# HyHuang1995/gmmloc

Hardware: AMD Instinct MI355X
Metric: frames/sec (associate+pose-refine), 2k pts x 4k GMM (higher is better)
Workload: dtype f64

## Files before the change

gmmloc_amd/csrc/gl_ba.hip:

```cpp
#include <algorithm>
#include <cstdlib>
#include <cstring>

#include "gl_ba_common.hpp"

#pragma clang fp contract(fast)

using namespace gld;
using namespace glba;

namespace {

GL_DEV void point_solve(const PtLin& o, double lambda, double* f, double* b, double* u) {
  double D[6];
#pragma unroll
  for (int i = 0; i < 6; ++i) D[i] = o.A[i] + o.Hc[i];
  D[0] += lambda;
  D[3] += lambda;
  D[5] += lambda;
  ldl3_factor(D, f);
#pragma unroll
  for (int i = 0; i < 3; ++i) b[i] = o.a[i] + o.bc[i];
  ldl3_solve(f, b, u);
}
// ... 380 lines not shown
    if (!pose_fixed) se3_store(T, pose_io + (size_t)f * 7);
    if (iters_out) iters_out[f] = it3;
  }
}

}

namespace gl {

bool ba1_fast_supported(int L);
int launch_ba1_fast(Ctx* c, const Gmm* g, const gl_camera* cam, const gl_params* prm, int B, int L, double* pose,
                    double* pts, const double* obs, const int32_t* oct, int32_t* assoc, const double* d2, double gate,
                    uint8_t* dropped, uint8_t* erase, int32_t* iters, char* scratch, const Ba1Layout& lay, const uint8_t* prior,
                    const TrackFixed* fixed);

int track_frames_fixed(gl_ctx_t* ctx, const gl_gmm_t* gmm, const gl_camera* cam, const gl_params* prm, int B, int M,
                       double* pose_dev, double* Xw_dev, const double* obs_dev, const int32_t* octave_dev, int32_t* assoc_dev,
                       double* d2_dev, const gl_track_anchor* anchor);

int launch_ba1(Ctx* c, const Gmm* g, const gl_camera* cam, const gl_params* prm, int B, int L, double* pose,
               const uint8_t* has_prior, double* pts, const double* obs, const int32_t* oct, int32_t* assoc,
               const double* d2, double gate, uint8_t* dropped, uint8_t* erase, int32_t* iters, char* scratch, const Ba1Layout& lay) {
  BaK k = make_bak(cam, prm, gate);
  GmmDev gm{g->rec12, g->axis, g->sqrt_info, g->hgw, g->flags, g->plane4};
  {
    TimerScope ts(c, GL_TIMER_BA);
    k_ba1<<<B, T_BA, 0, c->stream>>>(k, gm, B, L, pose, has_prior, pts, obs, oct, assoc, d2, (double*)(scratch + lay.trial),
                                     (double*)(scratch + lay.chi), (uint8_t*)(scratch + lay.lev), dropped, erase, iters);
  }
  GL_HIP(hipGetLastError());
  return GL_OK;
}

}

static int track_frames_impl(gl_ctx_t* ctx, const gl_gmm_t* gmm, const gl_camera* cam, const gl_params* prm, int B, int M,
                             double* pose_dev, double* Xw_dev, const double* obs_dev, const int32_t* octave_dev,
                             int32_t* assoc_dev, double* d2_dev, const uint8_t* prior_dev, const gl::TrackFixed* fixed = nullptr) {
  GL_REQUIRE(ctx && gmm && cam && prm, "null argument");
  if (B == 0 || M == 0) return GL_OK;
  GL_REQUIRE(B > 0 && M > 0, "bad B / M");
  GL_REQUIRE(pose_dev && Xw_dev && obs_dev && octave_dev && assoc_dev, "null buffer");
  gl::Ctx* c = gl::C(ctx);
  gl::Gmm* g = gl::G(gmm);
  GL_HIP(hipSetDevice(c->device));
  const size_t n = (size_t)B * M;
  const bool fast = (c->opt.ba_slow == 0 || fixed) && gl::ba1_fast_supported(M);
  gl::Ba1Layout lay;
  int rc = gl::ba1_layout(c, B, M, fixed ? fixed->F : 0, prior_dev != nullptr, fast, &lay);
  if (rc != GL_OK) return rc;
  const bool use_grid = g->grid.enabled && c->opt.assoc_grid != 0;
  const size_t assoc_bytes =
      use_grid ? gl::assoc_index_scratch_bytes(g->K, (int)n, d2_dev != nullptr) : gl::assoc_scratch_bytes(g->K, (int)n);
  gl::Regions r{0};
  r.take(std::max(assoc_bytes, lay.end));
  const size_t o_d2 = r.take(n * 8);
  void* scratch = nullptr;
  rc = gl::ctx_scratch(c, r.off, &scratch);
  if (rc != GL_OK) return rc;
  double* d2 = d2_dev ? d2_dev : (double*)((char*)scratch + o_d2);
  if (use_grid)
    rc = gl::launch_assoc_index(c, g, Xw_dev, (int)n, assoc_dev, d2, d2_dev != nullptr, scratch);
  else
    rc = gl::launch_assoc_brute(c, g, Xw_dev, (int)n, assoc_dev, d2);
  if (rc != GL_OK) return rc;
  if (fast)
    return gl::launch_ba1_fast(c, g, cam, prm, B, M, pose_dev, Xw_dev, obs_dev, octave_dev, assoc_dev, d2, 9.0,
                               nullptr, nullptr, nullptr, (char*)scratch, lay, prior_dev, fixed);
  return gl::launch_ba1(c, g, cam, prm, B, M, pose_dev, prior_dev, Xw_dev, obs_dev, octave_dev, assoc_dev, d2, 9.0,
                        nullptr, nullptr, nullptr, (char*)scratch, lay);
}

extern "C" int gl_track_frames(gl_ctx_t* ctx, const gl_gmm_t* gmm, const gl_camera* cam, const gl_params* prm, int B,
                               int M, double* pose_dev, double* Xw_dev, const double* obs_dev,
                               const int32_t* octave_dev, int32_t* assoc_dev, double* d2_dev) {
  return track_frames_impl(ctx, gmm, cam, prm, B, M, pose_dev, Xw_dev, obs_dev, octave_dev, assoc_dev, d2_dev, nullptr);
}

extern "C" int gl_track_frames_anchored(gl_ctx_t* ctx, const gl_gmm_t* gmm, const gl_camera* cam, const gl_params* prm, int B,
                                        int M, double* pose_dev, double* Xw_dev, const double* obs_dev,
                                        const int32_t* octave_dev, int32_t* assoc_dev, double* d2_dev,
                                        const gl_track_anchor* anchor) {
  GL_REQUIRE(anchor, "null anchor");
  GL_REQUIRE(anchor->F >= 0 && anchor->F <= GL_TRACK_MAX_FIXED, "bad number of fixed observer key-frames");
  if (anchor->F == 0)
    return track_frames_impl(ctx, gmm, cam, prm, B, M, pose_dev, Xw_dev, obs_dev, octave_dev, assoc_dev, d2_dev, anchor->prior_dev);
  GL_REQUIRE(anchor->fixed_pose_dev && anchor->fixed_obs_dev && anchor->fixed_oct_dev, "null buffer of the fixed observer key-frames");
  if (ctx && anchor->F <= 4 && gl::ba1_fast_supported(M) && gl::C(ctx)->opt.ba_fixed_pack == 0 && gl::C(ctx)->opt.ba_slow == 0) {
    const gl::TrackFixed fx{anchor->F, anchor->fixed_pose_dev, anchor->fixed_obs_dev, anchor->fixed_oct_dev, anchor->fixed_erase_dev};
    return track_frames_impl(ctx, gmm, cam, prm, B, M, pose_dev, Xw_dev, obs_dev, octave_dev, assoc_dev, d2_dev, anchor->prior_dev, &fx);
  }
  return gl::track_frames_fixed(ctx, gmm, cam, prm, B, M, pose_dev, Xw_dev, obs_dev, octave_dev, assoc_dev, d2_dev, anchor);
}

static int track_frame_host_impl(gl_ctx_t* ctx, const gl_gmm_t* gmm, const gl_camera* cam, const gl_params* prm, int M,
                                 double* pose_host, double* Xw_host, const double* obs_host, const int32_t* octave_host,
                                 int32_t* assoc_host, int with_prior) {
  GL_REQUIRE(ctx && gmm && cam && prm, "null argument");
  GL_REQUIRE(M >= 0, "bad M");
  if (M == 0) return GL_OK;
  GL_REQUIRE(pose_host && Xw_host && obs_host && octave_host && assoc_host, "null buffer");
  gl::Ctx* c = gl::C(ctx);
  GL_HIP(hipSetDevice(c->device));
  const size_t oX = 64, oA = oX + (size_t)M * 24, oO = oA + (((size_t)M * 4 + 7) / 8) * 8, oC = oO + (size_t)M * 24,
               total = oC + (size_t)M * 4;
  if (c->stage_bytes < total) {
    GL_HIP(hipStreamSynchronize(c->stream));
    if (c->dev_stage) GL_HIP(hipFree(c->dev_stage));
    if (c->host_stage) GL_HIP(hipHostFree(c->host_stage));
    c->dev_stage = c->host_stage = nullptr;
    c->stage_bytes = 0;
    const size_t want = total + total / 4 + 64;
    GL_HIP(hipMalloc(&c->dev_stage, want));
    GL_HIP(hipHostMalloc(&c->host_stage, want, hipHostMallocDefault));
    c->stage_bytes = want;
  }
  char* st = (char*)c->host_stage;
  char* dv = (char*)c->dev_stage;
  memcpy(st, pose_host, 56);
  st[56] = with_prior ? 1 : 0;
  memcpy(st + oX, Xw_host, (size_t)M * 24);
  memcpy(st + oO, obs_host, (size_t)M * 24);
// ... 28 lines not shown
```

gmmloc_amd/csrc/gl_ba_fast.hip:

```cpp
#include <algorithm>
#include <cstdlib>

#include "gl_ba_common.hpp"

using namespace gld;
using namespace glba;

namespace {
struct PrepView {
  double* gobn;
  int32_t* perm;
  int32_t* pfl;
  int32_t* assoc_p;
};
struct FixedV {
  int F;
  double* fRt;
  double* fobn;
  int32_t* foct;
  double* chif;
  uint8_t* ferase;
};
struct BafKArgs {
  glba::BaK k;
  glba::GmmDev gm;
  int B, L, G, S;
  double* pose_io;
  double* pts_io;
  int32_t* assoc_all;
  uint8_t* dropped_all;
  uint8_t* erase_all;
  int32_t* iters_out;
  double* pn_all;
  int32_t* trials_out;
  int NB;
  unsigned long long* parts;
  int* ctl;
  long long limit;
  int xcc_trusted;
  const int32_t* oct_all;
  const uint8_t* prior_all;
  double* prior_mi;
  double* stage;
  int nb_prev;
  int32_t* counters;
  int32_t* outer_out;
  FixedV fxv;
  int32_t* edges_out;
  int* frame_ctr;
};
__host__ __device__ inline PrepView prep_view(double* scratch, int B, int L) {
  PrepView v;
  const size_t n = (size_t)B * L;
  v.gobn = scratch;
  v.perm = (int32_t*)(scratch + n * 3);
  v.pfl = v.perm + n;
  v.assoc_p = v.pfl + n;
  return v;
}

constexpr int PREP_T = 256, PREP_C = 8;
__global__ __launch_bounds__(PREP_T) void k_ba1_prep(BafKArgs A, const double* __restrict__ obs_all, const double* __restrict__ d2_all,
                                                    gl::TrackFixed fin, int* __restrict__ frame_ctr) {
  __shared__ int cnt[PREP_C][PREP_T / 64];
  __shared__ int cnt0[PREP_C][PREP_T / 64];
  const BaK& k = A.k;
  const int B = A.B, L = A.L, F = A.fxv.F;
  const int32_t* const oct_all = A.oct_all;
  int32_t* const assoc_all = A.assoc_all;
  const int f = blockIdx.x, tid = threadIdx.x, lane = tid & 63, wave = tid >> 6;
  if (f >= B) return;
  if (f == 0 && tid == 0) *frame_ctr = 0;
  if (A.parts) {
    const int nxw = 2 * A.G * 64;
    for (int i = tid; i < nxw; i += PREP_T) A.parts[(size_t)f * nxw + i] = 0ull;
    if (tid < 2) A.ctl[2 * f + tid] = 0;
  }
  if (A.prior_all && A.prior_all[f] && tid == 0) {
    const SE3 Ti = se3_inverse(se3_load(A.pose_io + (size_t)f * 7));
    double Ri[9];
    qtoR(Ti.r, Ri);
#pragma unroll
    for (int i = 0; i < 9; ++i) A.prior_mi[(size_t)f * 12 + i] = Ri[i];
#pragma unroll
    for (int i = 0; i < 3; ++i) A.prior_mi[(size_t)f * 12 + 9 + i] = Ti.t[i];
  }
  if (F > 0 && tid < F) {
    const SE3 T = se3_load(fin.pose + ((size_t)f * F + tid) * 7);
    double Rm[9];
    qtoR(T.r, Rm);
    double* o = A.fxv.fRt + ((size_t)f * F + tid) * 12;
#pragma unroll
    for (int i = 0; i < 9; ++i) o[i] = Rm[i];
#pragma unroll
    for (int i = 0; i < 3; ++i) o[9 + i] = T.t[i];
  }
  const size_t gbase = (size_t)f * L;
  const PrepView pv = prep_view(A.pn_all, B, L);
  const int rounds = (L + PREP_T - 1) / PREP_T;
  int a_[PREP_C], fl_[PREP_C];
#pragma unroll
  for (int j = 0; j < PREP_C; ++j) {
// ... 26 lines not shown
  __syncthreads();
  int total = 0, total0 = 0;
#pragma unroll
  for (int j = 0; j < PREP_C; ++j)
#pragma unroll
    for (int w = 0; w < PREP_T / 64; ++w) {
      total += cnt[j][w];
      total0 += cnt0[j][w];
    }
  const int n_others = L - total - total0, n_exist = L - total0;
  const double ifx = 1.0 / k.fx, ify = 1.0 / k.fy;
  int base = 0, base0 = 0;
#pragma unroll
  for (int j = 0; j < PREP_C; ++j) {
#pragma unroll
    for (int w = 0; w < PREP_T / 64; ++w)
      if (w < wave) {
        base += cnt[j][w];
        base0 += cnt0[j][w];
      }
    const int l = j * PREP_T + tid;
    const bool isnd = (fl_[j] & 12) == 4;
    const bool isempty = fl_[j] == 0 && j < rounds && l < L;
    const unsigned long long bal = __ballot(isnd), bal0 = __ballot(isempty);
    const int before = base + __popcll(bal & ((1ull << lane) - 1ull));
    const int before0 = base0 + __popcll(bal0 & ((1ull << lane) - 1ull));
    if (j < rounds && l < L) {
      const int lp = isempty ? n_exist + before0 : isnd ? n_others + before : l - before - before0;
      const size_t g = gbase + l, gp = gbase + lp;
      pv.perm[gp] = l;
      pv.pfl[gp] = fl_[j];
      pv.assoc_p[gp] = a_[j];
      pv.gobn[gp * 3] = (obs_all[g * 3] - k.cx) * ifx;
      pv.gobn[gp * 3 + 1] = (obs_all[g * 3 + 1] - k.cy) * ify;
      pv.gobn[gp * 3 + 2] = (obs_all[g * 3 + 2] - k.cx) * ifx;
      for (int kf = 0; kf < F; ++kf) {
        const size_t src = g * F + kf, dst = ((size_t)f * F + kf) * L + lp;
        const int fo = fl_[j] ? fin.oct[src] : -1;
        const double u = fin.obs[src * 3], v = fin.obs[src * 3 + 1], ur = fin.obs[src * 3 + 2];
        A.fxv.fobn[dst * 3] = (u - k.cx) * ifx;
        A.fxv.fobn[dst * 3 + 1] = (v - k.cy) * ify;
        A.fxv.fobn[dst * 3 + 2] = (ur - k.cx) * ifx;
        A.fxv.foct[dst] = fo < 0 ? -1 : ((fo & 7) | (!(ur < 0) ? 16 : 0));
        A.fxv.chif[dst] = 0.0;
      }
    }
#pragma unroll
    for (int w = 0; w < PREP_T / 64; ++w)
      if (w >= wave) {
        base += cnt[j][w];
        base0 += cnt0[j][w];
      }
  }
}
}

namespace {
struct BafCfg {
  int mcap, nw;
  bool spread, step32, prior, fixed;
};
namespace bafd2000 { constexpr BafCfg kCfg{2000, 8, false, false, false, false}; }
namespace bafs { constexpr BafCfg kCfg{256, 8, true, false, false, false}; }
#ifndef GL_BAF_QUICK
namespace bafd496 { constexpr BafCfg kCfg{496, 2, false, false, false, false}; }
namespace bafd1000 { constexpr BafCfg kCfg{1000, 4, false, false, false, false}; }
namespace bafs32 { constexpr BafCfg kCfg{256, 8, true, true, false, false}; }
namespace bafd2000s32 { constexpr BafCfg kCfg{2000, 8, false, true, false, false}; }
namespace bafd496p { constexpr BafCfg kCfg{496, 2, false, false, true, false}; }
namespace bafd1000p { constexpr BafCfg kCfg{992, 4, false, false, true, false}; }
namespace bafd2000p { constexpr BafCfg kCfg{2000, 8, false, false, true, false}; }
namespace bafsp { constexpr BafCfg kCfg{256, 8, true, false, true, false}; }
namespace bafd496f { constexpr BafCfg kCfg{496, 2, false, false, true, true}; }
namespace bafd1000f { constexpr BafCfg kCfg{984, 4, false, false, true, true}; }
namespace bafd2000f { constexpr BafCfg kCfg{2000, 8, false, false, true, true}; }
#endif
}
#define GL_BAF_NS bafd2000
#include "gl_ba_fast_impl.hpp"
#define GL_BAF_NS bafs
#include "gl_ba_fast_impl.hpp"
#ifndef GL_BAF_QUICK
#define GL_BAF_NS bafd496
#include "gl_ba_fast_impl.hpp"
#define GL_BAF_NS bafd1000
#include "gl_ba_fast_impl.hpp"
#define GL_BAF_NS bafs32
#include "gl_ba_fast_impl.hpp"
#define GL_BAF_NS bafd2000s32
#include "gl_ba_fast_impl.hpp"
#define GL_BAF_NS bafd496p
#include "gl_ba_fast_impl.hpp"
#define GL_BAF_NS bafd1000p
#include "gl_ba_fast_impl.hpp"
#define GL_BAF_NS bafd2000p
#include "gl_ba_fast_impl.hpp"
#define GL_BAF_NS bafsp
#include "gl_ba_fast_impl.hpp"
#define GL_BAF_NS bafd496f
#include "gl_ba_fast_impl.hpp"
#define GL_BAF_NS bafd1000f
#include "gl_ba_fast_impl.hpp"
#define GL_BAF_NS bafd2000f
#include "gl_ba_fast_impl.hpp"
namespace {
__device__ __forceinline__ int xcc_id() { return __builtin_amdgcn_s_getreg(20 | (0 << 6) | (3 << 11)) & 15; }
// ... 126 lines not shown
  in->kern<<<grid, threads, in->lds, c->stream>>>(a);
  GL_HIP(hipGetLastError());
  return GL_OK;
}

static int launch_spread(Ctx* c, BafKArgs a) {
  const BafInst* in = baf_instance(c, true, a.prior_all != nullptr, 0, 64 * a.S);
  GL_REQUIRE(in, "no refine instance for this launch");
  GL_HIP(ensure_dynamic_lds(c, (const void*)in->kern, in->lds));
  a.NB = a.G;
  a.limit = (long long)(c->opt.ba_rendezvous_us * 100.0);
  if (c->opt.ba_test_abort_seq > 0) a.limit = -(long long)c->opt.ba_test_abort_seq;
  a.xcc_trusted = (c->xcc_ids_trusted && c->opt.ba_same_xcd != 0) ? 1 : 0;
  const int grid = a.NB > 1 ? 64 * ((a.B + 7) / 8) : a.B;
  in->kern<<<grid, 256, in->lds, c->stream>>>(a);
  GL_HIP(hipGetLastError());
  return GL_OK;
}

int launch_ba1_fast(Ctx* c, const Gmm* g, const gl_camera* cam, const gl_params* prm, int B, int L, double* pose,
                    double* pts, const double* obs, const int32_t* oct, int32_t* assoc, const double* d2, double gate,
                    uint8_t* dropped, uint8_t* erase, int32_t* iters, char* scratch, const Ba1Layout& lay, const uint8_t* prior,
                    const TrackFixed* fixed) {
  BafKArgs a{};
  a.k = make_bak(cam, prm, gate);
  a.gm = GmmDev{g->rec12, g->axis, g->sqrt_info, g->hgw, g->flags, g->plane4};
  a.B = B;
  a.L = L;
  canon_order(L, &a.G, &a.S);
  a.pose_io = pose;
  a.pts_io = pts;
  a.assoc_all = assoc;
  a.dropped_all = dropped;
  a.erase_all = erase;
  a.iters_out = iters;
  a.pn_all = (double*)(scratch + lay.rec);
  a.trials_out = (c->stats && c->stats_n >= B) ? c->stats : nullptr;
  a.NB = 1;
  a.oct_all = oct;
  a.prior_all = prior;
  a.prior_mi = (double*)(scratch + lay.prior_mi);
  a.counters = c->counters;
  a.outer_out = a.trials_out ? c->stats_iters : nullptr;
  if (fixed)
    a.fxv = FixedV{fixed->F, (double*)(scratch + lay.frt), (double*)(scratch + lay.fobn), (int32_t*)(scratch + lay.foct),
                   (double*)(scratch + lay.chif), fixed->erase};
  a.edges_out = (c->stats_edges && c->stats_edges_n >= B) ? c->stats_edges : nullptr;
  if (lay.spread) {
    a.parts = (unsigned long long*)(scratch + lay.parts);
    a.ctl = (int*)(scratch + lay.ctl);
    a.stage = (double*)(scratch + lay.stage);
  }
  int* const frame_ctr = (int*)(scratch + lay.frame_ctr);
  {
    TimerScope ts(c, GL_TIMER_BA_PREP);
    k_ba1_prep<<<B, PREP_T, 0, c->stream>>>(a, obs, d2, fixed ? *fixed : TrackFixed{}, frame_ctr);
  }
  GL_HIP(hipGetLastError());
  TimerScope ts(c, GL_TIMER_BA);
  if (!lay.spread) return launch_dense(c, a, frame_ctr);
  const int rc = launch_spread(c, a);
  if (rc != GL_OK || a.G == 1) return rc;
  a.nb_prev = a.G;
  return launch_dense(c, a, frame_ctr);
}

}
#endif
```

gmmloc_amd/csrc/gl_ba_fast_impl.hpp:

```cpp
namespace {
namespace GL_BAF_NS {

constexpr int MCAP = kCfg.mcap;
constexpr bool kSpread = kCfg.spread;
constexpr bool kStep32 = kCfg.step32;
constexpr bool kPrior = kCfg.prior;
constexpr bool kFixed = kCfg.fixed;
constexpr int NWC = kCfg.nw;
constexpr int NRED = kSpread ? 1 : NWC;
constexpr int TSP = 256;
constexpr bool kLean = !kPrior;

#ifdef GL_BA_TRACE
__device__ double g_trace[10 * 128];
#define TRACE_TRIAL(t, a, b, c_, d, dxp)                            \
  if (blockIdx.x == 0 && threadIdx.x == 0 && (t) < 128) {            \
    g_trace[(t)*10] = (a);                                           \
    g_trace[(t)*10 + 1] = (b);                                       \
    g_trace[(t)*10 + 2] = (c_);                                      \
    g_trace[(t)*10 + 3] = (d);                                       \
    for (int i_ = 0; i_ < 6; ++i_) g_trace[(t)*10 + 4 + i_] = (dxp)[i_]; \
  }
#else
#define TRACE_TRIAL(t, a, b, c_, d, dxp)
// ... 1582 lines not shown
    est[0] += est[2] * (trials - est[3]);
    est[1] += est[2] * cj;
  }
  return cj;
}

template <class T>
GL_DEV T ld_karg(const T __attribute__((address_space(4)))* p) {
  static_assert(sizeof(T) % 4 == 0, "");
  union U {
    T v;
    unsigned w[sizeof(T) / 4];
    GL_DEV U() {}
  } u;
  const unsigned __attribute__((address_space(4)))* q = (const unsigned __attribute__((address_space(4)))*)p;
#pragma unroll
  for (unsigned i = 0; i < sizeof(T) / 4; ++i) u.w[i] = q[i];
  return u.v;
}

GL_DEV bool false_once_inlined() { return false; }

constexpr int kPriorWorkOwn = (kPrior && !kSpread && NWC < 4) ? 108 : 0;
constexpr int kLdsSp = 0;
constexpr int kLdsChir = kLdsSp + 3 * MCAP;
constexpr int kLdsUn = kLdsChir + MCAP;
constexpr int kLdsRed = kLdsUn + 6 * MCAP;
constexpr int kLdsTot = kLdsRed + NRED * 32;
constexpr int kLdsStab = kLdsTot + 64;
constexpr int kLdsRed2 = kLdsStab + 24;
constexpr int kLdsPrec = kLdsRed2 + (NWC > 8 ? 2 * NWC : 16);
constexpr int kLdsFrt = kLdsPrec + (kPrior ? 64 : 0) + kPriorWorkOwn;
constexpr int kLdsTb = kLdsFrt + (kFixed ? kMaxFixed * 12 : 0);
constexpr size_t kLdsBytes = (kLdsTb + (kSpread ? 29 * TSP : 0)) * sizeof(double);

typedef const BafKArgs __attribute__((address_space(4))) kargs_t;
GL_DEV void ba1_fast_frame(double* smem, const unsigned fblock, kargs_t* ka) {
  const BaK __attribute__((address_space(4)))& k = ka->k;
  const GmmDev gm = ld_karg(&ka->gm);
  const FixedV fxv = ld_karg(&ka->fxv);
  const int B = ka->B, L = ka->L, G = ka->G, S = ka->S, NB = ka->NB, xcc_trusted = ka->xcc_trusted, nb_prev = ka->nb_prev;
  double* const pose_io = ka->pose_io;
  double* const pts_io = ka->pts_io;
  int32_t* const assoc_all = ka->assoc_all;
  double* const pn_all = ka->pn_all;
  unsigned long long* const parts = ka->parts;
  int* const ctl = ka->ctl;
  const long long limit = ka->limit;
  const int32_t* const oct_all = ka->oct_all;
  const uint8_t* const prior_all = ka->prior_all;
  const double* const prior_mi = ka->prior_mi;
  double* const stage = ka->stage;
  int32_t* const counters = ka->counters;
  Lds D;
  D.sp = smem + kLdsSp;
  D.chir = smem + kLdsChir;
  D.un = smem + kLdsUn;
  Red R;
  R.red = smem + kLdsRed;
  R.tot = smem + kLdsTot;
  D.stab = smem + kLdsStab;
  R.red2 = smem + kLdsRed2;
  double* const prec = smem + kLdsPrec;
  D.frt = smem + kLdsFrt;
  R.tb = smem + kLdsTb;
  double* const pwork = kSpread ? R.tb + 2 * TSP : (NWC >= 4 ? R.red : prec + 64);
  D.F = 0;
  D.Lf = L;
  D.gfobn = nullptr;
  D.gfoct = nullptr;
  D.gchif = nullptr;
  R.S = S;
  FlagW fw = {0ull, 0u};
  const int tid = threadIdx.x, lane = tid & 63, wave = tid >> 6;
  PROF_K(0);
#ifdef GL_BA_PROF
  if (blockIdx.x == 1024 && threadIdx.x == 0) g_prof_k[12] = 0;
  const unsigned long long prof_wg_t0 = wall_clock64();
#endif
  const int f = kSpread ? (NB > 1 ? (int)(fblock & 7) + 8 * (int)(fblock >> 6) : (int)fblock) : (int)fblock;
  const int pb_ = kSpread && NB > 1 ? (int)((fblock >> 3) & 7) : 0;
  if (f >= B || pb_ >= NB) return;
  double* const st_pts = stage;
  double* const st_pose = stage ? stage + (size_t)B * L * 3 : nullptr;
  int32_t* const st_assoc = stage ? (int32_t*)(st_pose + (size_t)B * 8) : nullptr;
  if (!kSpread && ctl) {
    if (ctl[2 * f + 1] == nb_prev) {
      const int32_t* oc = oct_all + (size_t)f * L;
      const int NT = blockDim.x;
      for (int l0 = threadIdx.x; l0 < L; l0 += 4 * NT) {
        int o_[4], a_[4];
        double p_[4][3];
#pragma unroll
        for (int q = 0; q < 4; ++q) {
          const int l = min(l0 + q * NT, L - 1);
          const size_t g = (size_t)f * L + l;
          o_[q] = oc[l];
          a_[q] = st_assoc[g];
#pragma unroll
          for (int j = 0; j < 3; ++j) p_[q][j] = st_pts[g * 3 + j];
        }
#pragma unroll
        for (int q = 0; q < 4; ++q) {
          const int l = l0 + q * NT;
          if (l >= L) break;
          const size_t g = (size_t)f * L + l;
// ... 2 lines not shown
            for (int j = 0; j < 3; ++j) pts_io[g * 3 + j] = p_[q][j];
          }
          assoc_all[g] = a_[q];
        }
      }
      if (threadIdx.x < 7) pose_io[(size_t)f * 7 + threadIdx.x] = st_pose[(size_t)f * 8 + threadIdx.x];
      return;
    }
    if (counters && threadIdx.x == 0) atomicAdd(&counters[0], 1);
  }
  Coop C{kSpread && NB > 1 ? parts + (size_t)f * 2 * NB * 64 : nullptr, kSpread ? NB : 1, pb_, 0u,
         ctl ? ctl + 2 * f : nullptr, (int*)(R.tot + 61), limit, 0, 0};
  Map mp;
  mp.L = L;
  if (kSpread) {
    mp.S = 1;
    mp.base = wave < S && C.pb < G ? (C.pb + G * wave) * 64 + lane : L;
    mp.lbase = tid;
    mp.step = 0;
  } else {
    mp.S = S;
    mp.base = wave * 64 + lane;
    mp.lbase = mp.base;
    mp.step = 64 * G;
  }
  const size_t gbase = (size_t)f * L;
  const PrepView pv = prep_view(pn_all, B, L);
  const double* gnd = gm.plane4;
  const double* gobn = pv.gobn + gbase * 3;
  const int32_t* gperm = pv.perm + gbase;
  const int32_t* gassoc = pv.assoc_p + gbase;
  const Uni U{uni(k.bf / k.fx), uni(k.ba_lambda2)};
  if (kFixed) {
    D.F = fxv.F;
    D.gfobn = fxv.fobn + (size_t)f * fxv.F * L * 3;
    D.gfoct = fxv.foct + (size_t)f * fxv.F * L;
    D.gchif = fxv.chif + (size_t)f * fxv.F * L;
    if (tid < fxv.F * 12) D.frt[tid] = fxv.fRt[(size_t)f * fxv.F * 12 + tid];
  }
  for (int i = tid; i < NRED * 32; i += blockDim.x) R.red[i] = 0.0;
  if (tid < (NWC > 8 ? 2 * NWC : 16)) R.red2[tid] = 0.0;
  if (tid == 0) {
    *(int*)(R.tot + 60) = 0;
    *(int*)(R.tot + 61) = 0;
    R.tot[62] = 0.0;
  }
  {
    const int ns = kSpread ? 1 : mp.S;
#pragma unroll 1
    for (int i = 0; i < ns; ++i) {
      const int l = mp.base + slot_off(mp, i), ll = mp.lbase + slot_off(mp, i);
      if (false_once_inlined()) continue;
      if (l >= L) break;
      const size_t g = gbase + gperm[l];
#pragma unroll
      for (int j = 0; j < 3; ++j) D.sp[j * MCAP + ll] = pts_io[g * 3 + j];
      D.chir[ll] = 0.0;
      fw_or(fw, i, pv.pfl[gbase + l] & 0xffff);
      if (kFixed) {
#pragma unroll
        for (int kf = 0; kf < kMaxFixed; ++kf)
          if (kf >= D.F || D.gfoct[(size_t)kf * L + l] < 0) fw_or(fw, i, F_OFFF << kf);
      }
      fw_activity(fw, i);
    }
  }
  PtConst pc;
  if (kSpread) load_const(mp, fw, gobn, gnd, gassoc, pc);
  if (tid == 0) {
#pragma unroll
    for (int j = 0; j < 8; ++j) {
      D.stab[j] = k.s2inv[j] * (k.fx * k.fx);
      D.stab[8 + j] = k.s2inv[j] * (k.fy * k.fy);
    }
    D.stab[16] = k.delta_mono;
    D.stab[17] = k.delta_mono * k.delta_mono;
    D.stab[18] = k.delta_stereo;
    D.stab[19] = k.delta_stereo * k.delta_stereo;
  }
  Pose P = pose_from_se3(se3_load(pose_io + (size_t)f * 7));
  const bool prior_flag = kPrior && prior_all ? prior_all[f] != 0 : false;
  Anchor An{prior_flag && k.first_as_prior != 0, prior_flag && k.first_as_prior == 0,
            (const cdouble_k*)(prior_mi + (size_t)f * 12), prec, 0, pwork, !kSpread && NWC >= 4,
            kSpread ? (int)(blockDim.x >> 6) - 1 : min(1, (int)(blockDim.x >> 6) - 1)};
  if (!kSpread && NWC == 8 && wave >= 4) __builtin_amdgcn_s_setprio(1);
  __syncthreads();
  if (kPrior && An.has_prior) {
    if (wave == An.wave) prior_record_wave(An.mi, P, prec, pwork, An.rezero);
    __syncthreads();
  }
  if (kSpread && C.NB > 1 && xcc_trusted) {
    double x2[32];
    const double id = (double)(__builtin_amdgcn_s_getreg(20 | (0 << 6) | (3 << 11)) & 15);
    x2[0] = id;
    x2[1] = id * id;
    reduce2<2>(x2, R, C);
    C.same_xcd = ((double)(C.NB * R.S * 64) * x2[1] == x2[0] * x2[0]) ? 1 : 0;
  }

  int it3 = 0, trials = 0, outer = 0;
  const int ns = kSpread ? 1 : mp.S;
  PROF_K(1);
#pragma unroll 1
  for (int phase = 0; phase < 3; ++phase) {
    it3 = optimize_fast(U, gm, D, mp, fw, P, gobn, gassoc, gnd, pc, phase < 2, phase < 2 ? 5 : 40, R, trials, C, An);
    outer += it3 > 0 ? it3 : 0;
    PROF_K(2 + 2 * phase);
    if (phase == 2) break;
#pragma unroll 1
    for (int i = 0; i < ns; ++i) {
      const int l = mp.base + slot_off(mp, i), ll = mp.lbase + slot_off(mp, i);
// ... 117 lines not shown
    }
#ifdef GL_BA_TRACE
    if (f == 0)
      for (int i = 0; i < 10 * 128 && i < L * 3; ++i) pts_io[i] = g_trace[i];
#endif
#ifdef GL_BA_PROF
    if (f == 0) {
      double* const pr = staged ? st_pose : pose_io;
      for (int i = 0; i < 7; ++i) pr[i] = (double)g_prof[i == 5 ? 7 : i];
    }
    if (f != 0 && f != 1024 && !kSpread) {
      pose_io[(size_t)f * 7] = (double)prof_wg_t0;
      pose_io[(size_t)f * 7 + 1] = (double)wall_clock64();
      pose_io[(size_t)f * 7 + 2] = (double)((__builtin_amdgcn_s_getreg(4 | (0 << 6) | (31 << 11)) & 0xffffff) | ((__builtin_amdgcn_s_getreg(20 | (0 << 6) | (3 << 11)) & 15) << 24));
      pose_io[(size_t)f * 7 + 3] = (double)trials;
    }
    if (f == 1024) {
      for (int i = 0; i < 7; ++i) pose_io[(size_t)f * 7 + i] = (double)g_prof_k[i];
      for (int i = 7; i < 13; ++i) pts_io[(size_t)f * L * 3 + (i - 7)] = (double)g_prof_k[i];
    }
    if (f == 0 && !staged) {
      for (int i = 0; i < 64 * 8 * 4 && i < L * 3; ++i) pts_io[i] = (double)g_prof_w[i];
      for (int i = 0; i < 16 * 8 * 2 * 5 && 2048 + i < L * 3; ++i) pts_io[2048 + i] = (double)g_prof_s[i];
      for (int i = 0; i < 10 * 8 * 2 * 4 * 3 && 2048 + 1280 + i < L * 3; ++i) pts_io[2048 + 1280 + i] = (double)g_prof_q[i];
    }
#endif
  }
  if (kSpread && C.ctl) {
    __syncthreads();
    if (tid == 0) __hip_atomic_fetch_add(C.ctl + 1, 1, __ATOMIC_RELAXED, __HIP_MEMORY_SCOPE_AGENT);
  }
  }
}

__global__ __launch_bounds__(kSpread ? TSP : 512, 2) void k_ba1_fast(BafKArgs A) {
  extern __shared__ __attribute__((aligned(16))) double smem[];
  __shared__ int s_frame;
  const bool persistent = !kSpread && A.frame_ctr != nullptr;
  bool first = true;
  kargs_t* ka = (kargs_t*)__builtin_amdgcn_kernarg_segment_ptr();
#pragma unroll 1
  for (;;) {
    asm volatile("" : "+s"(ka));
    unsigned fr = blockIdx.x;
    if (persistent) {
      if (threadIdx.x == 0) s_frame = atomicAdd(ka->frame_ctr, 1);
      __syncthreads();
      fr = (unsigned)s_frame;
      if ((int)fr >= ka->B) break;
    } else if (!first) {
      break;
    }
    first = false;
    ba1_fast_frame(smem, fr, ka);
    if (persistent) __syncthreads();
  }
}

}
}
#undef GL_BAF_NS
```

gmmloc_amd/csrc/gl_grid.hip:

```cpp
#include <algorithm>
#include <cmath>
#include <cstdlib>
#include <cstring>

#include <hipcub/hipcub.hpp>

#include "gl_device.hpp"
#include "gl_internal.hpp"

using namespace gld;

namespace {

struct GridDev {
  double lo[3];
  double inv_h;
  int dim[3];
  int nglob;
  double t_resolve;
  const int32_t* ptr;
  const int32_t* idx;
  const int32_t* glob;
  const int4* cell4;
  const unsigned long long* cell8;
};

GL_DEV int4 cell_unpack8(unsigned long long w) {
  if (w >> 63) return make_int4((int)((w >> 32) & 0x3fffffffull), (int)(w & 0xffffffffull), 0, 0);
  return make_int4((int)(w & 3ull), (int)((w >> 2) & 0xfffffull), (int)((w >> 22) & 0xfffffull), (int)((w >> 42) & 0xfffffull));
}
GL_DEV bool grid_packed(const GridDev& G) { return G.cell4 != nullptr || G.cell8 != nullptr; }
GL_DEV int4 cell_load(const GridDev& G, int c) { return G.cell8 ? cell_unpack8(G.cell8[c]) : G.cell4[c]; }

GL_DEV void upd_min(double d, int k, double& best, int& bi) {
  const bool take = (d < best) || (d == best && k < bi);
  best = take ? d : best;
  bi = take ? k : bi;
}

struct ArgMin {
  double d;
  int k;
};
GL_DEV ArgMin glob_min(const double* rec12, const GridDev& G, double x, double y, double z) {
  ArgMin m = {__builtin_inf(), 0x7fffffff};
  for (int j = 0; j < G.nglob; ++j) {
    const int k = G.glob[j];
    upd_min(chi2_srec((cdouble*)rec12 + (size_t)k * 12, x, y, z), k, m.d, m.k);
  }
  return m;
}

GL_DEV void store_min(const GridDev& G, int n, double best, int bi, int32_t* out_idx, double* out_d2, int32_t* rest_list,
                      int32_t* rest_count) {
  if (best <= G.t_resolve) {
    out_idx[n] = bi;
    if (out_d2) out_d2[n] = best;
  } else {
    out_idx[n] = -1;
    if (out_d2) out_d2[n] = __builtin_inf();
    if (rest_list) rest_list[atomicAdd(rest_count, 1)] = n;
  }
}

__global__ __launch_bounds__(256) void k_assoc_cells(const double* __restrict__ rec12, GridDev G,
                                                     const double* __restrict__ pts, int N,
                                                     int32_t* __restrict__ out_idx, double* __restrict__ out_d2,
                                                     int32_t* __restrict__ rest_list, int32_t* __restrict__ rest_count) {
  const int n = blockIdx.x * 256 + threadIdx.x;
  if (n >= N) return;
  const double x = pts[(size_t)n * 3], y = pts[(size_t)n * 3 + 1], z = pts[(size_t)n * 3 + 2];
  const ArgMin g0 = glob_min(rec12, G, x, y, z);
  double best = g0.d;
  int bi = g0.k;
  const double fx = (x - G.lo[0]) * G.inv_h, fy = (y - G.lo[1]) * G.inv_h, fz = (z - G.lo[2]) * G.inv_h;
  const bool inside = fx >= 0.0 && fx < (double)G.dim[0] && fy >= 0.0 && fy < (double)G.dim[1] && fz >= 0.0 &&
                      fz < (double)G.dim[2];
  if (inside) {
    const int c = ((int)fz * G.dim[1] + (int)fy) * G.dim[0] + (int)fx;
    if (grid_packed(G)) {
      const int4 q = cell_load(G, c);
      if (q.x <= 3) {
        if (q.x > 0) upd_min(chi2_rec(rec12 + (size_t)q.y * 12, x, y, z), q.y, best, bi);
        if (q.x > 1) upd_min(chi2_rec(rec12 + (size_t)q.z * 12, x, y, z), q.z, best, bi);
        if (q.x > 2) upd_min(chi2_rec(rec12 + (size_t)q.w * 12, x, y, z), q.w, best, bi);
      } else {
        for (int e = q.y; e < q.y + q.x; ++e) {
          const int k = G.idx[e];
          upd_min(chi2_rec(rec12 + (size_t)k * 12, x, y, z), k, best, bi);
        }
      }
    } else {
      const int e0 = G.ptr[c], e1 = G.ptr[c + 1];
      for (int e = e0; e < e1; ++e) {
        const int k = G.idx[e];
        upd_min(chi2_rec(rec12 + (size_t)k * 12, x, y, z), k, best, bi);
      }
    }
  }
  store_min(G, n, best, bi, out_idx, out_d2, rest_list, rest_count);
}

constexpr int CG_REC = 60;
constexpr int CG_LONE_LANES = 32;
constexpr int CG_TAG = 26, CG_KMASK = (1 << CG_TAG) - 1;
constexpr int CG_IDS = 304;
__global__ __launch_bounds__(256) void k_assoc_cells_coop(const double* __restrict__ rec12, const double* __restrict__ rec16, GridDev G,
                                                          const double* __restrict__ pts, int N,
                                                          int32_t* __restrict__ out_idx, double* __restrict__ out_d2,
// ... 472 lines not shown
  G.nglob = (int)glob.size();
  G.nnz = (size_t)nnz;
  G.ncell = ncell;
  G.cell4 = nullptr;
  G.cell8 = nullptr;
  const bool want8 = c->opt.assoc_cell8 != 0 && g->K < (1 << 20) && nnz < (1ll << 31);
  const double cell_bytes = want8 ? 8.0 : 16.0;
  if ((double)ncell * cell_bytes <= c->opt.assoc_pack_mb * 1048576.0) {
    void* tab = nullptr;
    if (hipMalloc(&tab, ncell * (size_t)cell_bytes) == hipSuccess) {
      if (want8) k_index_pack8<<<(unsigned)((ncell + 255) / 256), 256, 0, c->stream>>>(d_ptr, d_idx, ncell, (unsigned long long*)tab);
      else k_index_pack<<<(unsigned)((ncell + 255) / 256), 256, 0, c->stream>>>(d_ptr, d_idx, ncell, (int4*)tab);
      if (hipGetLastError() != hipSuccess || hipStreamSynchronize(c->stream) != hipSuccess) {
        (void)hipFree(tab);
        tab = nullptr;
      }
    } else {
      (void)hipGetLastError();
      tab = nullptr;
    }
    (want8 ? G.cell8 : G.cell4) = tab;
  }
  G.rec16 = nullptr;
  if (G.cell4 || G.cell8) {
    if (hipMalloc(&G.rec16, (size_t)g->K * 128) == hipSuccess) {
      k_rec_pad<<<(g->K * 16 + 255) / 256, 256, 0, c->stream>>>(g->rec12, g->K, G.rec16);
      if (hipGetLastError() != hipSuccess || hipStreamSynchronize(c->stream) != hipSuccess) {
        (void)hipFree(G.rec16);
        G.rec16 = nullptr;
      }
    } else {
      (void)hipGetLastError();
      G.rec16 = nullptr;
    }
  }
  G.enabled = true;
  return GL_OK;
}

static size_t index_list_bytes(int N) { return (((size_t)N * 4 + 64) + 63) / 64 * 64; }
size_t assoc_index_scratch_bytes(int K, int N, bool resolve_all) {
  return index_list_bytes(N) + (resolve_all ? assoc_scratch_bytes(K, N, true) : 0);
}

static GridDev grid_dev(const CellIndex& I) {
  GridDev G;
  for (int a = 0; a < 3; ++a) {
    G.lo[a] = I.lo[a];
    G.dim[a] = I.dim[a];
  }
  G.inv_h = I.inv_h;
  G.nglob = I.nglob;
  G.t_resolve = I.t_resolve;
  G.ptr = I.ptr;
  G.idx = I.idx;
  G.glob = I.glob;
  G.cell4 = (const int4*)I.cell4;
  G.cell8 = (const unsigned long long*)I.cell8;
  return G;
}

int launch_assoc_index(Ctx* c, const Gmm* g, const double* pts, int N, int32_t* idx, double* d2, bool resolve_all,
                       void* scratch) {
  const GridDev G = grid_dev(g->grid);
  int32_t* count = (int32_t*)scratch;
  int32_t* list = count + 16;
  TimerScope ts(c, GL_TIMER_ASSOC);
  if (resolve_all) GL_HIP(hipMemsetAsync(count, 0, 4, c->stream));
  int32_t* rl = resolve_all ? list : nullptr;
  const dim3 gr((N + 255) / 256);
  if ((G.cell4 || G.cell8) && g->grid.rec16 && g->K < (1 << 26) && N >= 4096 && c->opt.assoc_coop != 0)
    k_assoc_cells_coop<<<gr, 256, 0, c->stream>>>(g->rec12, g->grid.rec16, G, pts, N, idx, d2, rl, count);
  else
    k_assoc_cells<<<gr, 256, 0, c->stream>>>(g->rec12, G, pts, N, idx, d2, rl, count);
  GL_HIP(hipGetLastError());
  if (resolve_all)
    return launch_assoc_sweep(c, g, pts, N, idx, d2, list, count, (char*)scratch + index_list_bytes(N));
  return GL_OK;
}

}

extern "C" {

int gl_gmm_index_bytes(const gl_gmm_t* gmm, double bytes[3]) {
  GL_REQUIRE(gmm && bytes, "null argument");
  const gl::CellIndex& I = gl::G(gmm)->grid;
  bytes[0] = I.enabled ? (double)(I.ncell + 1) * 4.0 : 0.0;
  bytes[1] = I.enabled ? (double)I.nnz * 4.0 + (double)I.nglob * 4.0 : 0.0;
  bytes[2] = I.cell8 ? (double)I.ncell * 8.0 : I.cell4 ? (double)I.ncell * 16.0 : 0.0;
  return GL_OK;
}

int gl_gmm_index_info(const gl_gmm_t* gmm, double info[8]) {
  GL_REQUIRE(gmm && info, "null argument");
  const gl::CellIndex& I = gl::G(gmm)->grid;
  info[0] = I.enabled ? 1.0 : 0.0;
  info[1] = I.h;
  info[2] = I.dim[0];
  info[3] = I.dim[1];
  info[4] = I.dim[2];
  info[5] = (double)I.nnz;
  info[6] = I.nglob;
  info[7] = I.t_resolve;
  return GL_OK;
}

int gl_assoc_index_work(gl_ctx_t* ctx, const gl_gmm_t* gmm, const double* pts_dev, int N, int64_t* pairs_dev) {
  GL_REQUIRE(ctx && gmm && pairs_dev, "null argument");
  gl::Ctx* c = gl::C(ctx);
  gl::Gmm* g = gl::G(gmm);
  GL_HIP(hipSetDevice(c->device));
  GL_HIP(hipMemsetAsync(pairs_dev, 0, 8, c->stream));
  if (N == 0 || !g->grid.enabled) return GL_OK;
  GL_REQUIRE(N > 0 && pts_dev, "bad N / pts");
  k_index_work<<<(N + 255) / 256, 256, 0, c->stream>>>(gl::grid_dev(g->grid), pts_dev, N, (unsigned long long*)pairs_dev);
  GL_HIP(hipGetLastError());
// ... 5 lines not shown
```

gmmloc_amd/csrc/gl_internal.hpp:

```cpp
#pragma once
#include <hip/hip_runtime.h>
#include <stdint.h>

#include <map>
#include <string>
#include <tuple>
#include <vector>

#include "gmmloc_hip.h"

namespace gl {

void set_error(const char* fmt, ...);

#define GL_HIP(expr)                                                                  \
  do {                                                                                \
    hipError_t _e = (expr);                                                           \
    if (_e != hipSuccess) {                                                           \
      gl::set_error("%s:%d: %s -> %s", __FILE__, __LINE__, #expr, hipGetErrorString(_e)); \
      return GL_ERR_DEVICE;                                                           \
    }                                                                                 \
  } while (0)

#define GL_REQUIRE(cond, msg)              \
// ... 204 lines not shown
void free_cell_index(Gmm* g);
struct PoseCompacted;
int pose_compacted_launch(gl_ctx_t* ctx, const gl_camera* cam, const gl_params* prm, int B, int M, double* pose_dev, const double* Xw_dev,
                          const double* obs_dev, const int32_t* octave_dev, uint8_t* outlier_dev, int32_t* ninlier_dev, int nin_stride,
                          const PoseCompacted& pc);
int optimize_current_pose_plain(gl_ctx_t* ctx, const gl_camera* cam, const gl_params* prm, int B, int M, double* pose_dev, const double* Xw_dev,
                                const double* obs_dev, const int32_t* octave_dev, uint8_t* outlier_dev, int32_t* ninlier_dev, int nin_stride);
int launch_bow_gated(gl_ctx_t* ctx, float nn_ratio, int check_orientation, int B, int N1, int N2, int NN1, int NN2, const float* angle1_dev,
                     const uint8_t* desc1_dev, const uint8_t* has_mp1_dev, const int32_t* nnode1_dev, const int32_t* node_id1_dev,
                     const int32_t* node_ptr1_dev, const int32_t* node_idx1_dev, const float* angle2_dev, const uint8_t* desc2_dev,
                     const int32_t* nnode2_dev, const int32_t* node_id2_dev, const int32_t* node_ptr2_dev, const int32_t* node_idx2_dev,
                     int32_t* match21_dev, int32_t* nmatches_dev, const int32_t* run_flag);
int launch_match_frame_gated(gl_ctx_t* ctx, const gl_camera* cam, float scale_factor, int B, int NF, int NL, const double* pose_cw, const double* pose_lw,
                             const double* feat_uv, const float* feat_ur, const int32_t* feat_oct, const float* feat_angle, const uint8_t* feat_desc,
                             const uint8_t* feat_taken, const double* last_pt, const uint8_t* last_valid, const int32_t* last_oct, const float* last_angle,
                             const uint8_t* last_desc, float th, int mono, int check_orientation, int32_t* feat_match, int32_t* nmatches,
                             const int32_t* gate_nm, int gate_min);
struct LocalMapDerive {
  int32_t* match_last;
  int32_t* match_kf;
  const int32_t* last_mp;
  const int32_t* kf_feat_mp;
  const int32_t* counts2;
  int NL, NK;
};
struct LocalMapLists {
  int KFcap, NPcap;
  int32_t *feat_mp, *local_kf, *n_local_kf, *local_mp, *n_local_mp, *ref_kf, *kf_count, *status;
};
struct LocalMapGathered {
  double *mp_pos, *mp_normal;
  float *mp_max_dist, *mp_min_dist;
  uint8_t *mp_cand, *mp_desc;
  int32_t *last_to_local, *kf_to_local;
};
int local_map_check(const gl_map_view* map, int B, int NF, const LocalMapLists& L, bool need_point_arrays);
size_t local_map_scratch_bytes(const Ctx* c, const gl_map_view* map, int B, bool have_kf_count);
int local_map_launch(Ctx* c, const gl_map_view* map, int B, int NF, const LocalMapLists& L, const LocalMapDerive* derive, void* scratch);
size_t local_map_gathered_place(void* base, int B, int NPcap, int NL, int NK, LocalMapGathered* out);
int local_map_gather_launch(Ctx* c, const gl_map_view* map, int B, int NL, int NK, const LocalMapLists& L, const int32_t* last_mp,
                            const int32_t* kf_feat_mp, const LocalMapGathered& G);
int launch_assoc_brute(Ctx* c, const Gmm* g, const double* pts, int N, int32_t* idx, double* d2);
int launch_assoc_sweep(Ctx* c, const Gmm* g, const double* pts, int N, int32_t* idx, double* d2, const int32_t* list,
                       const int32_t* count_dev, void* scratch);
size_t assoc_scratch_bytes(int K, int N, bool listed = false);
inline int sweep_points(int N, bool listed) { return listed ? (N / 16 > 256 ? N / 16 : 256) : N; }
void sweep_split(int K, int N, bool listed, int ppt, int* ptiles, int* nsplit, int* kchunk);
int build_screen_records(Ctx* c, Gmm* g);
int launch_assoc_screened(Ctx* c, const Gmm* g, const double* pts, int N, int32_t* idx, double* d2, const int32_t* list,
                          const int32_t* count_dev);
int launch_assoc_sweep64(Ctx* c, const Gmm* g, const double* pts, int N, int32_t* idx, double* d2, const int32_t* list,
                         const int32_t* count_dev, void* scratch);
int launch_assoc_index(Ctx* c, const Gmm* g, const double* pts, int N, int32_t* idx, double* d2, bool resolve_all,
                       void* scratch);
size_t assoc_index_scratch_bytes(int K, int N, bool resolve_all);

#ifdef __HIPCC__
namespace mapdev {
__device__ __forceinline__ bool mp_ok(const gl_map_view& m, int p) { return p >= 0 && p < m.NMP && (!m.mp_valid || m.mp_valid[p]); }
__device__ __forceinline__ bool kf_ok(const gl_map_view& m, int k) { return !m.kf_valid || m.kf_valid[k]; }
__device__ __forceinline__ void obs_range(const gl_map_view& m, int p, int* o0, int* o1) {
  const int a = m.obs_ptr[p], b = m.obs_ptr[p + 1];
  const bool ok = a >= 0 && b >= a && b <= m.NOBS;
  *o0 = ok ? a : 0;
  *o1 = ok ? b : 0;
}
template <int T, class V>
__device__ __forceinline__ V block_excl_scan(V v, V* s_w, int tid, V* total) {
  const int lane = tid & 63, w = tid >> 6;
  V inc = v;
#pragma unroll
  for (int o = 1; o < 64; o <<= 1) {
    const V t = __shfl_up(inc, o);
    if (lane >= o) inc += t;
  }
  if (lane == 63) s_w[w] = inc;
  __syncthreads();
  V base = 0, tot = 0;
#pragma unroll
  for (int i = 0; i < T / 64; ++i) {
    const V x = s_w[i];
    base += i < w ? x : 0;
    tot += x;
  }
  __syncthreads();
  *total = tot;
  return base + inc - v;
}
typedef unsigned long long u64;
constexpr int SCAN_T = 1024, SCAN_PER = 4, SCAN_TILE = SCAN_T * SCAN_PER;
__device__ __forceinline__ void tile_scan(u64* cnt, u64* tile, size_t n, u64* s_w, int tid, int b) {
  const size_t base = (size_t)b * SCAN_TILE + (size_t)tid * SCAN_PER;
  u64 v[SCAN_PER], sum = 0;
#pragma unroll
  for (int u = 0; u < SCAN_PER; ++u) {
    v[u] = base + u < n ? cnt[base + u] : 0ull;
    sum += v[u];
  }
  u64 total;
  u64 at = block_excl_scan<SCAN_T, u64>(sum, s_w, tid, &total);
#pragma unroll
  for (int u = 0; u < SCAN_PER; ++u) {
    if (base + u < n) cnt[base + u] = at;
    at += v[u];
  }
  if (tid == 0) tile[b] = total;
}
// ... 17 lines not shown
```

Baseline: 411,700.

## Fuse BA prep into persistent BA kernel and gate associations at grid store

The separate k_ba1_prep launch is replaced, for the non-spread, no-prior, no-fixed path, by a per-frame record builder that runs inside the persistent BA kernel and writes points and flags straight into LDS. The grid association kernel can now apply the chi2 gate when it stores, so the d2 buffer is neither written nor read in that case. This removes one kernel launch and a global round trip of the permuted records and d2. In exchange it adds LDS staging, extra block barriers per frame and more code in the main kernel, which may raise register pressure.

```diff
diff --git a/gmmloc_amd/csrc/gl_ba.hip b/gmmloc_amd/csrc/gl_ba.hip
--- a/gmmloc_amd/csrc/gl_ba.hip
+++ b/gmmloc_amd/csrc/gl_ba.hip
@@ -456,22 +456,24 @@
   const bool use_grid = g->grid.enabled && c->opt.assoc_grid != 0;
   const size_t assoc_bytes =
       use_grid ? gl::assoc_index_scratch_bytes(g->K, (int)n, d2_dev != nullptr) : gl::assoc_scratch_bytes(g->K, (int)n);
+  const double gate = 9.0;
+  const bool gate_at_store = use_grid && fast && !d2_dev;
   gl::Regions r{0};
   r.take(std::max(assoc_bytes, lay.end));
-  const size_t o_d2 = r.take(n * 8);
+  const size_t o_d2 = (d2_dev || gate_at_store) ? 0 : r.take(n * 8);
   void* scratch = nullptr;
   rc = gl::ctx_scratch(c, r.off, &scratch);
   if (rc != GL_OK) return rc;
-  double* d2 = d2_dev ? d2_dev : (double*)((char*)scratch + o_d2);
+  double* d2 = d2_dev ? d2_dev : gate_at_store ? nullptr : (double*)((char*)scratch + o_d2);
   if (use_grid)
-    rc = gl::launch_assoc_index(c, g, Xw_dev, (int)n, assoc_dev, d2, d2_dev != nullptr, scratch);
+    rc = gl::launch_assoc_index(c, g, Xw_dev, (int)n, assoc_dev, d2, d2_dev != nullptr, scratch, gate_at_store ? gate : -1.0);
   else
     rc = gl::launch_assoc_brute(c, g, Xw_dev, (int)n, assoc_dev, d2);
   if (rc != GL_OK) return rc;
   if (fast)
-    return gl::launch_ba1_fast(c, g, cam, prm, B, M, pose_dev, Xw_dev, obs_dev, octave_dev, assoc_dev, d2, 9.0,
+    return gl::launch_ba1_fast(c, g, cam, prm, B, M, pose_dev, Xw_dev, obs_dev, octave_dev, assoc_dev, d2, gate,
                                nullptr, nullptr, nullptr, (char*)scratch, lay, prior_dev, fixed);
-  return gl::launch_ba1(c, g, cam, prm, B, M, pose_dev, prior_dev, Xw_dev, obs_dev, octave_dev, assoc_dev, d2, 9.0,
+  return gl::launch_ba1(c, g, cam, prm, B, M, pose_dev, prior_dev, Xw_dev, obs_dev, octave_dev, assoc_dev, d2, gate,
                         nullptr, nullptr, nullptr, (char*)scratch, lay);
 }
 
diff --git a/gmmloc_amd/csrc/gl_ba_fast.hip b/gmmloc_amd/csrc/gl_ba_fast.hip
--- a/gmmloc_amd/csrc/gl_ba_fast.hip
+++ b/gmmloc_amd/csrc/gl_ba_fast.hip
@@ -48,6 +48,9 @@
   FixedV fxv;
   int32_t* edges_out;
   int* frame_ctr;
+  const double* obs_all;
+  const double* d2_all;
+  int make_rec;
 };
 __host__ __device__ inline PrepView prep_view(double* scratch, int B, int L) {
   PrepView v;
@@ -180,6 +183,134 @@
         base0 += cnt0[j][w];
       }
   }
+}
+
+typedef const BafKArgs __attribute__((address_space(4))) BafKArgsK;
+constexpr int MKR_C = 4, MKR_W = 8;
+__device__ __noinline__ void ba1_make_records(BafKArgsK* ka, const int f, double* sp, double* chir, double* stg, const int mcap, int* cnt,
+                                              const int NT, const int tid) {
+  int* const cnt0 = cnt + MKR_C * MKR_W;
+  const int B = ka->B, L = ka->L;
+  const double gate = ka->k.gate_chi2, cx = ka->k.cx, cy = ka->k.cy;
+  const double ifx = 1.0 / ka->k.fx, ify = 1.0 / ka->k.fy;
+  const double* const obs_all = ka->obs_all;
+  const double* const d2_all = ka->d2_all;
+  const int32_t* const oct_all = ka->oct_all;
+  const int32_t* const assoc_all = ka->assoc_all;
+  const double* const pts_io = ka->pts_io;
+  const uint8_t* const gflags = ka->gm.flags;
+  const PrepView pv = prep_view(ka->pn_all, B, L);
+  const int NW = __builtin_amdgcn_readfirstlane(NT) >> 6, lane = tid & 63, wave = __builtin_amdgcn_readfirstlane(tid >> 6);
+  const size_t gbase = (size_t)f * L;
+  int oc_[MKR_C], a_[MKR_C], fl_[MKR_C];
+  double d2_[MKR_C];
+  const bool gated = d2_all && gate >= 0;
+#pragma unroll
+  for (int j = 0; j < MKR_C; ++j) {
+    const size_t g = gbase + min(j * NT + tid, L - 1);
+    oc_[j] = oct_all[g];
+    a_[j] = assoc_all[g];
+    d2_[j] = 0.0;
+    if (gated) d2_[j] = d2_all[g];
+  }
+#pragma unroll
+  for (int j = 0; j < MKR_C; ++j) {
+    const int l = min(j * NT + tid, L - 1);
+    const size_t g = gbase + l;
+    double v[6];
+#pragma unroll
+    for (int c = 0; c < 3; ++c) {
+      v[c] = pts_io[g * 3 + c];
+      v[3 + c] = obs_all[g * 3 + c];
+    }
+#pragma unroll
+    for (int c = 0; c < 6; ++c) stg[c * mcap + l] = v[c];
+  }
+  __builtin_amdgcn_sched_barrier(0);
+#pragma unroll
+  for (int j = 0; j < MKR_C; ++j) {
+    int a = a_[j];
+    if (gated && !(d2_[j] <= gate)) a = -1;
+    if (oc_[j] < 0) a = -1;
+    a_[j] = a;
+  }
+  int deg_[MKR_C];
+#pragma unroll
+  for (int j = 0; j < MKR_C; ++j) deg_[j] = gflags[max(a_[j], 0)] & 1;
+  __builtin_amdgcn_sched_barrier(0);
+#pragma unroll
+  for (int j = 0; j < MKR_C; ++j) {
+    const int l = j * NT + tid;
+    const bool in = l < L;
+    const int oc = oc_[j], a = a_[j];
+    const int ex = oc >= 0 ? 1 : 0, as = (oc >= 0 && a >= 0) ? 1 : 0;
+    const int st = !(stg[5 * mcap + min(l, L - 1)] < 0) ? 2 : 0;
+    const int fl = ex * (1 | ((oc & 7) << 8) | st) | as * (4 | (deg_[j] << 3));
+    fl_[j] = in ? fl : 0;
+    a_[j] = in ? a : -1;
+    const unsigned long long bal = __ballot((fl_[j] & 12) == 4);
+    const unsigned long long bal0 = __ballot(fl_[j] == 0 && in);
+    if (lane == 0) {
+      cnt[j * MKR_W + wave] = __popcll(bal);
+      cnt0[j * MKR_W + wave] = __popcll(bal0);
+    }
+    if (wave == 0 && lane >= NW && lane < MKR_W) {
+      cnt[j * MKR_W + lane] = 0;
+      cnt0[j * MKR_W + lane] = 0;
+    }
+  }
+  __syncthreads();
+  __builtin_amdgcn_sched_barrier(0);
+  int base_[MKR_C], base0_[MKR_C], total = 0, total0 = 0;
+  {
+    int4 q[2 * MKR_C], q0[2 * MKR_C];
+#pragma unroll
+    for (int i = 0; i < 2 * MKR_C; ++i) {
+      q[i] = ((const int4*)cnt)[i];
+      q0[i] = ((const int4*)cnt0)[i];
+    }
+#pragma unroll
+    for (int j = 0; j < MKR_C; ++j) {
+      const int v[MKR_W] = {q[2 * j].x, q[2 * j].y, q[2 * j].z, q[2 * j].w, q[2 * j + 1].x, q[2 * j + 1].y, q[2 * j + 1].z, q[2 * j + 1].w};
+      const int v0[MKR_W] = {q0[2 * j].x, q0[2 * j].y, q0[2 * j].z, q0[2 * j].w, q0[2 * j + 1].x, q0[2 * j + 1].y, q0[2 * j + 1].z, q0[2 * j + 1].w};
+      base_[j] = total;
+      base0_[j] = total0;
+#pragma unroll
+      for (int w = 0; w < MKR_W; ++w) {
+        base_[j] += w < wave ? v[w] : 0;
+        base0_[j] += w < wave ? v0[w] : 0;
+        total += v[w];
+        total0 += v0[w];
+      }
+    }
+  }
+  __builtin_amdgcn_sched_barrier(0);
+  const int n_others = L - total - total0, n_exist = L - total0;
+#pragma unroll
+  for (int j = 0; j < MKR_C; ++j) {
+    const int l = j * NT + tid;
+    const bool isnd = (fl_[j] & 12) == 4;
+    const bool isempty = fl_[j] == 0 && l < L;
+    const unsigned long long bal = __ballot(isnd), bal0 = __ballot(isempty);
+    const int before = base_[j] + __popcll(bal & ((1ull << lane) - 1ull));
+    const int before0 = base0_[j] + __popcll(bal0 & ((1ull << lane) - 1ull));
+    if (l < L) {
+      const int lp = isempty ? n_exist + before0 : isnd ? n_others + before : l - before - before0;
+      const size_t gp = gbase + lp;
+      double v[6];
+#pragma unroll
+      for (int c = 0; c < 6; ++c) v[c] = stg[c * mcap + l];
+      pv.perm[gp] = l;
+      pv.assoc_p[gp] = a_[j];
+      pv.gobn[gp * 3] = (v[3] - cx) * ifx;
+      pv.gobn[gp * 3 + 1] = (v[4] - cy) * ify;
+      pv.gobn[gp * 3 + 2] = (v[5] - cx) * ifx;
+#pragma unroll
+      for (int c = 0; c < 3; ++c) sp[c * mcap + lp] = v[c];
+      *(int*)(chir + lp) = fl_[j];
+    }
+  }
+  __syncthreads();
 }
 }
 
@@ -412,9 +543,16 @@
     a.stage = (double*)(scratch + lay.stage);
   }
   int* const frame_ctr = (int*)(scratch + lay.frame_ctr);
+  const bool make_rec = !lay.spread && a.fxv.F == 0 && !prior;
+  a.obs_all = obs;
+  a.d2_all = d2;
+  a.make_rec = make_rec ? 1 : 0;
   {
     TimerScope ts(c, GL_TIMER_BA_PREP);
-    k_ba1_prep<<<B, PREP_T, 0, c->stream>>>(a, obs, d2, fixed ? *fixed : TrackFixed{}, frame_ctr);
+    if (make_rec)
+      GL_HIP(hipMemsetAsync(frame_ctr, 0, sizeof(int), c->stream));
+    else
+      k_ba1_prep<<<B, PREP_T, 0, c->stream>>>(a, obs, d2, fixed ? *fixed : TrackFixed{}, frame_ctr);
   }
   GL_HIP(hipGetLastError());
   TimerScope ts(c, GL_TIMER_BA);
diff --git a/gmmloc_amd/csrc/gl_ba_fast_impl.hpp b/gmmloc_amd/csrc/gl_ba_fast_impl.hpp
--- a/gmmloc_amd/csrc/gl_ba_fast_impl.hpp
+++ b/gmmloc_amd/csrc/gl_ba_fast_impl.hpp
@@ -1658,6 +1658,7 @@
   const double* const prior_mi = ka->prior_mi;
   double* const stage = ka->stage;
   int32_t* const counters = ka->counters;
+  const int make_rec = ka->make_rec;
   Lds D;
   D.sp = smem + kLdsSp;
   D.chir = smem + kLdsChir;
@@ -1766,11 +1767,15 @@
       const int l = mp.base + slot_off(mp, i), ll = mp.lbase + slot_off(mp, i);
       if (false_once_inlined()) continue;
       if (l >= L) break;
-      const size_t g = gbase + gperm[l];
-#pragma unroll
-      for (int j = 0; j < 3; ++j) D.sp[j * MCAP + ll] = pts_io[g * 3 + j];
+      if (!kSpread && !kPrior && make_rec) {
+        fw_or(fw, i, *(const int*)(D.chir + ll) & 0xffff);
+      } else {
+        const size_t g = gbase + gperm[l];
+#pragma unroll
+        for (int j = 0; j < 3; ++j) D.sp[j * MCAP + ll] = pts_io[g * 3 + j];
+        fw_or(fw, i, pv.pfl[gbase + l] & 0xffff);
+      }
       D.chir[ll] = 0.0;
-      fw_or(fw, i, pv.pfl[gbase + l] & 0xffff);
       if (kFixed) {
 #pragma unroll
         for (int kf = 0; kf < kMaxFixed; ++kf)
@@ -1994,6 +1999,13 @@
       break;
     }
     first = false;
+    if (!kSpread && !kPrior) {
+      if (ka->make_rec && (int)fr < ka->B) {
+        double* sm = smem;
+        asm volatile("" : "+v"(sm));
+        ba1_make_records(ka, (int)fr, sm + kLdsSp, sm + kLdsChir, sm + kLdsUn, MCAP, (int*)(sm + kLdsRed), (int)blockDim.x, (int)threadIdx.x);
+      }
+    }
     ba1_fast_frame(smem, fr, ka);
     if (persistent) __syncthreads();
   }
diff --git a/gmmloc_amd/csrc/gl_grid.hip b/gmmloc_amd/csrc/gl_grid.hip
--- a/gmmloc_amd/csrc/gl_grid.hip
+++ b/gmmloc_amd/csrc/gl_grid.hip
@@ -18,6 +18,7 @@
   int dim[3];
   int nglob;
   double t_resolve;
+  double gate;
   const int32_t* ptr;
   const int32_t* idx;
   const int32_t* glob;
@@ -54,7 +55,7 @@
 GL_DEV void store_min(const GridDev& G, int n, double best, int bi, int32_t* out_idx, double* out_d2, int32_t* rest_list,
                       int32_t* rest_count) {
   if (best <= G.t_resolve) {
-    out_idx[n] = bi;
+    out_idx[n] = best <= G.gate ? bi : -1;
     if (out_d2) out_d2[n] = best;
   } else {
     out_idx[n] = -1;
@@ -633,6 +634,7 @@
   G.inv_h = I.inv_h;
   G.nglob = I.nglob;
   G.t_resolve = I.t_resolve;
+  G.gate = __builtin_inf();
   G.ptr = I.ptr;
   G.idx = I.idx;
   G.glob = I.glob;
@@ -642,8 +644,12 @@
 }
 
 int launch_assoc_index(Ctx* c, const Gmm* g, const double* pts, int N, int32_t* idx, double* d2, bool resolve_all,
-                       void* scratch) {
-  const GridDev G = grid_dev(g->grid);
+                       void* scratch, double gate) {
+  GridDev G = grid_dev(g->grid);
+  if (gate >= 0) {
+    GL_REQUIRE(!resolve_all, "the gate at the store is for callers that do not resolve the rest");
+    G.gate = gate;
+  }
   int32_t* count = (int32_t*)scratch;
   int32_t* list = count + 16;
   TimerScope ts(c, GL_TIMER_ASSOC);
diff --git a/gmmloc_amd/csrc/gl_internal.hpp b/gmmloc_amd/csrc/gl_internal.hpp
--- a/gmmloc_amd/csrc/gl_internal.hpp
+++ b/gmmloc_amd/csrc/gl_internal.hpp
@@ -280,7 +280,7 @@
 int launch_assoc_sweep64(Ctx* c, const Gmm* g, const double* pts, int N, int32_t* idx, double* d2, const int32_t* list,
                          const int32_t* count_dev, void* scratch);
 int launch_assoc_index(Ctx* c, const Gmm* g, const double* pts, int N, int32_t* idx, double* d2, bool resolve_all,
-                       void* scratch);
+                       void* scratch, double gate = -1.0);
 size_t assoc_index_scratch_bytes(int K, int N, bool resolve_all);
 
 #ifdef __HIPCC__
```

After: 414,200, median of 6. No clear change (+0.6%).
